# Hippogriff/prifit

Measured on AMD Instinct MI355X. Metric: shapes/sec (fwd+bwd) B=24x2048 pts, PointNet++-MSG+ellipsoid fit, higher is better.
Workload: dtype f32; 1 GPU; configs[2]: PointNet++-MSG + mean-shift(10 it, <=25 clusters) + ellipsoid fit + convex loss, B=24x2048 per GPU, fwd+bwd+Adam; global_batch=24, points=2048, parallelism=dp1, cloud=blobs, embedding=clustered, backbone_grad_param=sa1.conv_blocks.0.0.weight, launch=eager

## Files before the change

### include/prifit_hip.h

```cpp
#ifndef PRIFIT_HIP_H
#define PRIFIT_HIP_H

#include <stdint.h>

#ifdef __cplusplus
extern "C" {
#endif

#define PRIFIT_OK 0
#define PRIFIT_EINVAL (-1)
#define PRIFIT_ELAUNCH (-2)

#define PRIFIT_ABI_VERSION 200
int prifit_version(const char **arch);


int prifit_fps(const float *xyz, int B, int N, int npoint, const int64_t *start_idx,
               int64_t *out_idx, float *new_xyz, void *stream);

int prifit_ball_query(const float *xyz, const float *new_xyz, int B, int N, int S, int R,
                      const float *radius2, const int *nsample, void *const *out, int idx64,
                      void *stream);

int prifit_three_nn(const float *xyz1, const float *xyz2, int B, int N, int S, int32_t *idx,
                    float *dist, float *weight, void *stream);

int prifit_square_distance(const float *src, const float *dst, int B, int S, int N, float *out,
                           void *stream);


int prifit_group_gather(const float *feat, const float *xyz, const float *new_xyz,
                        const int32_t *idx, int B, int N, int S, int K, int C, int order,
                        int ld_out, float *out, void *stream);

int prifit_group_scatter_add(const float *gout, int ld_gout, int col0, const int32_t *idx, int B,
                             int N, int S, int K, int C, float *dfeat, void *stream);

int prifit_pack_cols(const float *w, int rows, int src_cols, const int32_t *map, int dst_cols, float *out, void *stream);
int prifit_unpack_cols(const float *g, int rows, int dst_cols, const int32_t *inv_off, const int32_t *inv_idx, int src_cols,
                       float *gw, void *stream);
int prifit_pack_cols_max_jobs(void);
int prifit_pack_cols_multi(int njobs, const float *const *w, const int32_t *rows, const int32_t *src_cols, const int32_t *const *map,
                           const int32_t *dst_cols, float *const *out, void *stream);
int prifit_unpack_cols_multi(int njobs, const float *const *g, const int32_t *rows, const int32_t *dst_cols, const int32_t *const *inv_off,
                             const int32_t *const *inv_idx, const int32_t *src_cols, float *const *gw, void *stream);

int prifit_three_interpolate(const float *points2, const int32_t *idx, const float *weight, int B,
                             int N, int S, int C, int ld_out, int col0, float *out, void *stream);

int prifit_three_interpolate_bwd(const float *gout, int ld_gout, int col0, const int32_t *idx,
                                 const float *weight, int B, int N, int S, int C, float *dpoints2,
                                 void *stream);
int prifit_fp_rows(const float *points2, const int32_t *idx, const float *weight, const float *points1, int B, int N, int S, int D2,
                   int D1, int kp, float *out, void *stream);


#define PRIFIT_GEMM_NT 0
#define PRIFIT_GEMM_NN 1
#define PRIFIT_GEMM_TN 2
#define PRIFIT_EPI_NONE 0
#define PRIFIT_EPI_CHORD 1
#define PRIFIT_EPI_MSKERNEL 2
#define PRIFIT_EPI_MSBWD 3

int prifit_gemm_f32(int layout, int M, int N, int K, const float *A, long long lda, long long strideA,
                    const float *B, long long ldb, long long strideB, float *C, long long ldc,
                    long long strideC, int batch, int splitk, const float *a_scale,
                    const float *a_shift, const float *b_scale, const float *b_shift,
                    const float *bias, long long bias_batch_stride, float *col_stats, int epilogue,
                    const float *epi_batch_scalar, const float *epi_aux, long long ld_aux,
                    long long stride_aux, const float *epi_row_add, float *a_rowsum, int accumulate, void *stream);

int prifit_chord_sym_f32(const float *A, long long lda, long long strideA, float *C, long long ldc, long long strideC,
                         int n, int K, int batch, unsigned long long *owner_key, void *stream);
int prifit_chord_sym_mask(const float *A, long long lda, long long strideA, const float *thr, uint32_t *mask, int n, int K, int batch,
                          unsigned long long *owner_key, void *stream);
int prifit_gram_sym_f32(const float *A, long long lda, long long strideA, float *C, long long ldc, long long strideC, int n, int K,
                        int batch, void *stream);

int prifit_gemm_pool_f32(int M, int N, int K, const float *A, long long lda, const float *W, long long ldb, float *Y,
                         long long ldc, const float *a_scale, const float *a_shift, const float *bias, float *col_stats,
                         float *cand, void *stream);
int prifit_gemm_pool_supported(int M, int N, int K);

int prifit_gemm_stream_f32(int layout, int M, int N, int K, const float *A, long long lda, const float *B,
                           long long ldb, float *C, long long ldc, const float *a_scale, const float *a_shift,
                           const float *bias, float *col_stats, void *stream);
int prifit_gemm_stream_supported(int layout, int M, int N, int K);
int prifit_gemm_stream_slabs(int M, int K);

int prifit_gemm_dual_nn_f32(int M, int N, int K1, int K2, const float *A1, const float *A2, long long lda,
                            long long strideA, const float *B1, const float *B2, long long ldb, long long strideB,
                            float *C, long long ldc, long long strideC, int batch, int splitk, int accumulate,
                            void *stream);

int prifit_gemm_dgrad_bnred_f32(int M, int N, int K, const float *dY, long long lda, const float *W, long long ldb,
                                float *G, long long ldc, const float *Yprev, long long ldy, const float *scale,
                                const float *shift, const float *mean, const float *invstd, float *red_slab, void *stream);
int prifit_slab_sum(const float *part, int nslab, long long n, float *out, void *stream);
int prifit_global_pool_winners_supported(int Cout, int Cin);
int prifit_global_pool_winners_f32(int Bs, int K, int Cout, int Cin, const int32_t *arg, const float *T, const float *W,
                                   long long ldw, const float *X, long long ldx, float *dX, long long lddx, float *dW,
                                   long long lddw, void *stream);

int prifit_gemm_stream_gather_f32(int M, int N, const int32_t *idx, const float *U, const float *Vc, int n_points, int n_centres,
                                  int rows_per_centre, const float *B, long long ldb, float *C, long long ldc,
                                  const float *a_scale, const float *a_shift, const float *bias, float *col_stats, void *stream);
int prifit_gemm_stream_bwd_gather_f32(long long P, int Cout, const float *G, const float *Y, const float *scale,
                                      const float *shift, const float *coef_a, const float *coef_b, const float *coef_d,
                                      const float *W, long long ldw, const int32_t *idx, const float *U, const float *Vc,
                                      int n_points, int n_centres, int rows_per_centre, const float *p_scale,
                                      const float *p_shift, const float *p_mean, const float *p_invstd, float *Gp, long long ldgp,
                                      float *red_slab, float *dW, long long lddw, float *workspace, void *stream);
int prifit_gemm_stream_pool_f32(int M, int N, int K, const float *A, long long lda, const float *B, long long ldb,
                                float *C, long long ldc, const float *a_scale, const float *a_shift, const float *bias,
                                float *col_stats, float *cand, void *stream);
int prifit_pool_from_candidates(const float *cand, const float *scale, const float *shift, int G, int K, int C,
                                int rows_per_sample, float slope, float *out, long long ldo, int32_t *arg, float *ystar,
                                void *stream);

int prifit_gemm_stream_dgrad_f32(int M, int N, int K, const float *dY, long long lda, const float *W, long long ldb,
                                 float *G, long long ldc, const float *Yprev, long long ldy, const float *scale,
                                 const float *shift, const float *mean, const float *invstd, float *red_slab, void *stream);

int prifit_pool_bwd_table(const float *gp, long long ldgp, const float *Y, long long ldy, const int32_t *arg,
                          const float *scale, const float *shift, const float *coef_a, int G, int K, int C, float slope,
                          float *T, void *stream);
int prifit_gemm_stream_dgrad_pool_f32(int M, int N, int K, const float *Y, long long lda, const float *W, long long ldb,
                                      float *G, long long ldc, const float *bias_dW, const int32_t *pool_arg,
                                      const float *pool_T, const float *coef_b, int pool_K, const float *Yprev,
                                      long long ldy, const float *scale, const float *shift, const float *mean,
                                      const float *invstd, float *red_slab, void *stream);
int prifit_gemm_stream_tn_pool_f32(int Mo, int No, long long P, const float *Y, long long ldy, const float *A,
                                   long long lda, float *out, long long ldo, const float *b_scale,
                                   const float *b_shift, const int32_t *pool_arg, const float *pool_T,
                                   const float *coef_b, const float *coef_d, int pool_K, float *workspace,
                                   void *stream);

int prifit_gemm_stream_tn_bn_f32(int Mo, int No, long long P, const float *G, const float *Y, long long ldy, const float *A,
                                 long long lda, float *out, long long ldo, const float *b_scale, const float *b_shift,
                                 const float *scale, const float *shift, const float *coef_a, const float *coef_b,
                                 const float *coef_d, float *workspace, void *stream);
int prifit_gemm_stream_dgrad_bn_f32(int M, int N, int K, const float *Gin, const float *Y, long long lda, const float *W,
                                    long long ldb, float *G, long long ldc, const float *scale_l, const float *shift_l,
                                    const float *coef_a, const float *coef_b, const float *coef_d, const float *Yprev,
                                    long long ldy, const float *scale, const float *shift, const float *mean,
                                    const float *invstd, float *red_slab, void *stream);
int prifit_gemm_stream_tn_f32(int Mo, int No, long long P, const float *G, long long ldg, const float *A,
                              long long lda, float *out, long long ldo, const float *b_scale,
                              const float *b_shift, float *workspace, void *stream);
long long prifit_gemm_stream_tn_workspace(int Mo, int No, long long P);
int prifit_gemm_stream_tn_supported(int Mo, int No, long long P);

int prifit_gemm_tile_m(int N);
int prifit_gemm_stats_tile_m(int M, int N);


int prifit_reduce_rows_per_slab(void);
int prifit_pool_reduce_groups_per_slab(void);

int prifit_col_stats(const float *Y, long long ld, int P, int C, float *slab, void *stream);
long long prifit_col_sum_workspace(int P, int C);
int prifit_col_sum(const float *Y, long long ld, int P, int C, float *out, float *workspace, void *stream);
int prifit_col_sum_samples(const float *Y, long long ld, int P, int C, int rows_per_sample, float *out, float *workspace,
                           void *stream);

// ... 291 lines not shown
```

### prifit_amd/csrc/gemm.hip

```cpp
#include <stdlib.h>

#include <type_traits>

#include "common.h"

typedef float f32x16 __attribute__((ext_vector_type(16)));

enum { LAY_NT = 0, LAY_NN = 1, LAY_TN = 2 };
enum { EPI_NONE = 0, EPI_CHORD = 1, EPI_MSKERNEL = 2, EPI_MSBWD = 3, EPI_BNRED = 4 };

struct GemmArgs {
    const float *A, *B;
    float *C;
    int M, N, K;
    long long lda, ldb, ldc;
    long long sA, sB, sC;
    int batch, splitk;
    const float *a_scale, *a_shift;
    const float *b_scale, *b_shift;
    const float *bias;
    long long bias_stride;
    float *stats;
    int epi;
    const float *epi_batch_scalar;
    const float *aux;
    const float *row_add;
    float *a_rowsum;
    long long ldaux, sAux;
    const float *red_scale, *red_shift, *red_mean, *red_invstd;
    long long dA2, dB2;
    int kswitch;
    int accumulate;
    int vecA, vecB;
    int ntiles;
    float *cand;
};

#ifndef GEMM_W8
#define GEMM_W8 6
#endif
constexpr int BK = 32;
constexpr int PAD = 4;

__device__ __forceinline__ float4 ld4(const float *p) { return *reinterpret_cast<const float4 *>(p); }

template <int ROWS, bool KC, bool VEC, bool AFF, int NTH>
struct TileLoader {
    static constexpr int NV = ROWS * BK / 4 / NTH;
    static_assert(NV * NTH * 4 == ROWS * BK, "tile must divide evenly over the threads");
    float4 v[NV];
    const float *ptr[NV];
    int klo[NV];
    int c0[NV];
    unsigned okmask[NV];
    long long step;
    int K, R, cclamp;

    __device__ __forceinline__ void init(const float *__restrict__ base, long long ld, int r0, int R_, int K_)
    {
        K = K_; R = R_;
        step = KC ? (long long)BK : (long long)BK * ld;
#pragma unroll
        for (int p = 0; p < NV; ++p) {
            const int id = threadIdx.x + NTH * p;
            if (KC) {
                const int gr = r0 + id / (BK / 4);
                klo[p] = (id % (BK / 4)) * 4;
                okmask[p] = gr < R ? 0xFu : 0u;
                ptr[p] = base + (long long)(gr < R ? gr : 0) * ld + (klo[p] < K ? klo[p] : 0);
                c0[p] = 0;
            } else {
                klo[p] = id / (ROWS / 4);
                const int gr = r0 + (id % (ROWS / 4)) * 4;
                unsigned m = 0;
#pragma unroll
                for (int j = 0; j < 4; ++j) m |= (gr + j < R) ? (1u << j) : 0u;
                okmask[p] = m;
                c0[p] = m ? gr : 0;
                ptr[p] = base + (long long)klo[p] * ld + c0[p];
            }
        }
    }

    int kload;
    __device__ __forceinline__ void load(int k0, const float *__restrict__, const float *__restrict__)
    {
        kload = k0;
        const int kt = k0 / BK;
#pragma unroll
        for (int p = 0; p < NV; ++p) {
            const int gk = k0 + klo[p];
            const bool kin = gk < K;
            const float *src = ptr[p] + (kin ? (long long)kt * step : 0);
            if (!KC && !kin && klo[p] >= K) src = ptr[p] - (long long)klo[p] * (step / BK);
            if (VEC) {
                v[p] = ld4(src);
            } else {
                float e[4];
#pragma unroll
                for (int j = 0; j < 4; ++j) {
                    const bool ok = KC ? (okmask[p] && (gk + j) < K) : (kin && ((okmask[p] >> j) & 1u));
                    e[j] = src[ok ? j : 0];
                }
                v[p] = make_float4(e[0], e[1], e[2], e[3]);
            }
        }
    }

    __device__ __forceinline__ void finish(const float *__restrict__ scale, const float *__restrict__ shift)
    {
#pragma unroll
        for (int p = 0; p < NV; ++p) {
            const int gk = kload + klo[p];
            const bool kin = gk < K;
            float4 x = v[p];
            if (VEC) {
                if (AFF) {
                    const int cc = KC ? (kin ? gk : 0) : c0[p];
                    const float4 s = ld4(scale + cc), t = ld4(shift + cc);
                    x.x = fmaxf(fmaf(x.x, s.x, t.x), 0.f); x.y = fmaxf(fmaf(x.y, s.y, t.y), 0.f);
                    x.z = fmaxf(fmaf(x.z, s.z, t.z), 0.f); x.w = fmaxf(fmaf(x.w, s.w, t.w), 0.f);
                }
                if (!(kin && okmask[p])) x = make_float4(0.f, 0.f, 0.f, 0.f);
            } else {
// ... 607 lines not shown
            const int y_voff = (RED && cok) ? (int)(((long long)rbase * g.ldaux + col) * 4) : 0x7fffffff;
            float kf[16];
            if (RED) {
#pragma unroll
                for (int r = 0; r < 16; ++r) {
                    const int ro = ((r & 3) + 8 * (r >> 2)) * ldy4;
                    kf[r] = __builtin_bit_cast(float, full_rows ? __builtin_amdgcn_raw_buffer_load_b32(yrs, y_voff, ro, 0)
                                                                 : __builtin_amdgcn_raw_buffer_load_b32(yrs, cok ? y_voff + ro : y_voff, 0, 0));
                }
            }
            float vmax = -INFINITY, vmin = INFINITY, v0 = 0.f;
            int imax = 0, imin = 0;
#pragma unroll
            for (int r = 0; r < 16; ++r) {
                const int row = rbase + (r & 3) + 8 * (r >> 2);
                const float v = acc[b][r] + bias;
                const float vs = (cok && (full_rows || row < g.M)) ? v : 0.f;
                if (PMAX) {
                    const int ri = (r & 3) + 8 * (r >> 2) + 4 * lh;
                    const bool rok = full_rows || row < g.M;
                    if (rok && v > vmax) { vmax = v; imax = ri; }
                    if (rok && v < vmin) { vmin = v; imin = ri; }
                }
                if (RED) {
                    const float gm = fmaf(kf[r], rs, rt) > 0.f ? vs : 0.f;
                    csum[b] += gm;
                    csq[b] += gm * ((kf[r] - rmu) * ris);
                } else {
                    csum[b] += vs;
                    if (r == 0) v0 = vs;
                    else if (r == 1) csq[b] = fmaf(v0, v0, vs * vs);
                    else csq[b] = fmaf(vs, vs, csq[b]);
                }
                {
                    const int ro = ((r & 3) + 8 * (r >> 2)) * ldc4;
                    if (full_rows) __builtin_amdgcn_raw_buffer_store_b32(__builtin_bit_cast(unsigned, v), crs, c_voff, ro, 0);
                    else __builtin_amdgcn_raw_buffer_store_b32(__builtin_bit_cast(unsigned, v), crs, cok ? c_voff + ro : c_voff, 0, 0);
                }
            }
            if (PMAX) {
                const float ov = __shfl_xor(vmax, 32, 64), on = __shfl_xor(vmin, 32, 64);
                const int oi = __shfl_xor(imax, 32, 64), oj = __shfl_xor(imin, 32, 64);
                if (ov > vmax || (ov == vmax && oi < imax)) { vmax = ov; imax = oi; }
                if (on < vmin || (on == vmin && oj < imin)) { vmin = on; imin = oj; }
                const int blk_row = m0 + wm0;
                if (lh == 0 && cok && blk_row < g.M) {
                    float *cd = g.cand + (long long)(blk_row >> 5) * 4 * g.N + col;
                    cd[0] = vmax; cd[g.N] = __int_as_float(imax); cd[2 * g.N] = vmin; cd[3 * g.N] = __int_as_float(imin);
                }
            }
        }
        PERS_STAMP(3);
        if (g.stats) {
            float *red = lds;
#pragma unroll
            for (int b = 0; b < TN; ++b) {
                const float s = csum[b] + __shfl_xor(csum[b], 32, 64);
                const float q = csq[b] + __shfl_xor(csq[b], 32, 64);
                if (lh == 0) {
                    red[(wmi * 2 + 0) * BN + wn0 + 32 * b + li] = s;
                    red[(wmi * 2 + 1) * BN + wn0 + 32 * b + li] = q;
                }
            }
            __syncthreads();
            for (int t = threadIdx.x; t < 2 * BN; t += NTH) {
                const int which = t / BN, c = t - which * BN;
                float s = 0.f;
#pragma unroll
                for (int w = 0; w < BM / WM; ++w) s += red[(w * 2 + which) * BN + c];
                if (n0 + c < g.N) g.stats[((long long)tile_m * 2 + which) * g.N + n0 + c] = s;
            }
            if (has_next) __syncthreads();
        }
        PERS_STAMP(4);
        if (!has_next) break;
        tix = ntix; tile_m = ntile_m; tile_n = ntile_n;
        la.finish(g.a_scale, g.a_shift);
        la.store(lds); lb.store(lds + SZA);
        __syncthreads();
        PERS_STAMP(5);
#ifdef PERS_STAMPS
        ++st_tile;
#endif
    }
}

#ifndef CHORD_XCD
#define CHORD_XCD 1
#endif
template <int MODE>
__global__ __launch_bounds__(512) __attribute__((amdgpu_waves_per_eu(4, 4))) void chord_sym_kernel(
    const float *__restrict__ A, long long lda, long long sA, float *__restrict__ C, long long ldc, long long sC, int n, int K,
    int batch, unsigned long long *__restrict__ okey, const float *__restrict__ thr, unsigned *__restrict__ mask)
{
    constexpr bool GRAM = MODE == 1, MASK = MODE == 2;
    constexpr int BM = 128, BN = 128, WM = 32, WN = 64, NTH = 512, TN = WN / 32, WAVES_N = BN / WN;
    constexpr int SZ = BM * (BK + PAD);
    constexpr int TLD = BM + 4;
    __shared__ __attribute__((aligned(16))) float lds[4 * SZ];
    static_assert(4 * SZ >= BN * TLD, "the transposed tile fits the staging buffers");
    const int T = n / BM;
    int t, zb;
#if CHORD_XCD
    xcd_shape_block((int)blockIdx.x, T * (T + 1) / 2, batch, zb, t);
#else
    t = (int)blockIdx.x % (T * (T + 1) / 2); zb = (int)blockIdx.x / (T * (T + 1) / 2);
#endif
    int tile_m = 0;
    while (t >= T - tile_m) { t -= T - tile_m; ++tile_m; }
    const int tile_n = tile_m + t;
    const int m0 = tile_m * BM, n0 = tile_n * BN;
    const float *Az = A + (long long)zb * sA;
    float *Cz = MASK ? nullptr : C + (long long)zb * sC;
    const int MW = n / 32;
    unsigned *Mz = MASK ? mask + (long long)zb * n * MW : nullptr;
    const float th = MASK ? thr[zb] : 0.f;
    const int wave = __builtin_amdgcn_readfirstlane(threadIdx.x >> 6), lane = threadIdx.x & 63;
    const int li = lane & 31, lh = lane >> 5;
    const int wm0 = (wave / WAVES_N) * WM, wn0 = (wave % WAVES_N) * WN;

    BufLoader<BM, true, false, NTH> la, lb;
    la.init(Az, lda, m0, n, K);
    lb.init(Az, lda, n0, n, K);
    const int ktiles = K / BK;
    la.load(0); lb.load(0);
    la.store(lds); lb.store(lds + SZ);
    __syncthreads();
    f32x16 acc[TN];
#pragma unroll
    for (int b = 0; b < TN; ++b)
#pragma unroll
        for (int r = 0; r < 16; ++r) acc[b][r] = 0.f;
    for (int kt = 0; kt < ktiles; ++kt) {
        const int stage = kt & 1;
        const float *As = lds + stage * 2 * SZ, *Bs = As + SZ;
        const bool more = kt + 1 < ktiles;
        if (more) { la.load((kt + 1) * BK); lb.load((kt + 1) * BK); }
#pragma unroll
        for (int gk = 0; gk < BK / 8; ++gk) {
            const float4 fa = read_frag<BM, true>(As, wm0 + li, gk, lh);
            float4 fb[TN];
#pragma unroll
            for (int b = 0; b < TN; ++b) fb[b] = read_frag<BN, true>(Bs, wn0 + 32 * b + li, gk, lh);
#pragma unroll
            for (int b = 0; b < TN; ++b) {
                acc[b] = __builtin_amdgcn_mfma_f32_32x32x2f32(fa.x, fb[b].x, acc[b], 0, 0, 0);
                acc[b] = __builtin_amdgcn_mfma_f32_32x32x2f32(fa.y, fb[b].y, acc[b], 0, 0, 0);
                acc[b] = __builtin_amdgcn_mfma_f32_32x32x2f32(fa.z, fb[b].z, acc[b], 0, 0, 0);
                acc[b] = __builtin_amdgcn_mfma_f32_32x32x2f32(fa.w, fb[b].w, acc[b], 0, 0, 0);
            }
        }
        if (more) {
            float *An = lds + (stage ^ 1) * 2 * SZ;
            la.store(An); lb.store(An + SZ);
        }
        __syncthreads();
    }
    const bool mirror = tile_m != tile_n;
    unsigned long long *okz = okey ? okey + (long long)zb * n : nullptr;
    auto fkey = [](float f) { const unsigned u = __float_as_uint(f); return (u & 0x80000000u) ? ~u : (u | 0x80000000u); };
#pragma unroll
    for (int b = 0; b < TN; ++b) {
        const int col = wn0 + 32 * b + li;
        float cmin = INFINITY;
        int cidx = 0;
#pragma unroll
// ... 82 lines not shown
#pragma unroll
        for (int r = 0; r < 16; ++r) acc[b][r] = 0.f;
    auto step = [&](int kt, auto par) {
        constexpr int S = decltype(par)::value;
        const float *As = lds + S * (SZA + SZB), *Bs = As + SZA;
        if (kt + 2 < kt1) { la[S].load((kt + 2) * BK); lb[S].load((kt + 2) * BK); }
        __builtin_amdgcn_sched_barrier(0);
        mma_ktile<BM, false, BN, false, TN>(As, Bs, wm0 + li, wn0 + li, lh, acc, BK / 8, nbv);
        if (kt + 1 < kt1) {
            float *An = lds + (S ^ 1) * (SZA + SZB);
            lb[S ^ 1].finish(g.b_scale, g.b_shift);
            la[S ^ 1].store(An); lb[S ^ 1].store(An + SZA);
        }
        __syncthreads();
    };
    int kt = kt0;
    for (; kt + 1 < kt1; kt += 2) {
        step(kt, std::integral_constant<int, 0>());
        step(kt + 1, std::integral_constant<int, 1>());
    }
    if (kt < kt1) step(kt, std::integral_constant<int, 0>());
    const int rbase = m0 + wm0 + 4 * lh;
#pragma unroll
    for (int b = 0; b < TN; ++b) {
        const int col = n0 + wn0 + 32 * b + li;
        if (col >= g.N) continue;
#pragma unroll
        for (int r = 0; r < 16; ++r) {
            const int row = rbase + (r & 3) + 8 * (r >> 2);
            if (row >= g.M) continue;
            float *dst = g.C + (long long)row * g.ldc + col;
            if (g.splitk > 1) unsafeAtomicAdd(dst, acc[b][r]);
            else if (g.accumulate) *dst += acc[b][r];
            else *dst = acc[b][r];
        }
    }
}

static bool launch_tnsk(const GemmArgs &g, hipStream_t st)
{
    if (g.batch != 1 || g.a_scale || g.bias || g.stats || g.epi != EPI_NONE || g.a_rowsum || g.kswitch ||
        !(g.vecA && g.vecB) || (g.M & 3) || (g.N & 3) || (g.splitk > 1 && !g.accumulate) || g.splitk > 65535)
        return false;
    const long long lim = 0x7ff00000LL;
    if ((long long)g.K * g.lda * 4 >= lim || (long long)g.K * g.ldb * 4 >= lim) return false;
    const dim3 grid(((g.M + 127) / 128) * ((g.N + 127) / 128), 1, g.splitk), block(512);
    if (g.b_scale) hipLaunchKernelGGL((gemm_tnsk_kernel<true>), grid, block, 0, st, g);
    else hipLaunchKernelGGL((gemm_tnsk_kernel<false>), grid, block, 0, st, g);
    return true;
}

static bool launch_persistent(const GemmArgs &g_, int lay, hipStream_t st, float *want_cand = nullptr, bool dry = false)
{
    GemmArgs g = g_;
    if (lay == LAY_TN || g.batch != 1 || g.splitk != 1 || g.accumulate || g.a_rowsum || g.kswitch ||
        g.b_scale || !(g.epi == EPI_NONE || g.epi == EPI_BNRED) || !(g.vecA && g.vecB) || (g.K & 3) || (lay == LAY_NN && (g.N & 3)))
        return false;
    const long long lim = 0x7ff00000LL;
    if ((long long)g.M * g.lda * 4 >= lim || (long long)(lay == LAY_NT ? g.N : g.K) * g.ldb * 4 >= lim ||
        (long long)g.M * g.ldc * 4 >= lim || (g.epi == EPI_BNRED && (long long)g.M * g.ldaux * 4 >= lim))
        return false;
    g.ntiles = ((g.M + 127) / 128) * ((g.N + 127) / 128);
    const int slots = 512;
    if (g.ntiles <= slots) return false;
    if (dry) return lay == LAY_NT && g.epi == EPI_NONE && g.a_scale;
    const dim3 grid(slots), block(512);
    if (lay == LAY_NT) {
        if (g.epi != EPI_NONE) return false;
        if (want_cand) {
            g.cand = want_cand;
            if (g.a_scale) hipLaunchKernelGGL((gemm_pers_kernel<LAY_NT, true, false, true>), grid, block, 0, st, g);
            else hipLaunchKernelGGL((gemm_pers_kernel<LAY_NT, false, false, true>), grid, block, 0, st, g);
        } else if (g.a_scale) hipLaunchKernelGGL((gemm_pers_kernel<LAY_NT, true, false>), grid, block, 0, st, g);
        else hipLaunchKernelGGL((gemm_pers_kernel<LAY_NT, false, false>), grid, block, 0, st, g);
    } else {
        if (want_cand) return false;
        if (g.a_scale) return false;
        if (g.epi == EPI_BNRED) hipLaunchKernelGGL((gemm_pers_kernel<LAY_NN, false, true>), grid, block, 0, st, g);
        else hipLaunchKernelGGL((gemm_pers_kernel<LAY_NN, false, false>), grid, block, 0, st, g);
    }
    return true;
}

__global__ __launch_bounds__(512, 4) void gemm_dual_sk_kernel(const GemmArgs g)
{
    constexpr int BM = 128, BN = 128, WN = 64, NTH = 512, TN = 2, WAVES_N = 2;
    constexpr int SZA = BM * (BK + PAD), SZB = BK * (BN + PAD);
    __shared__ __attribute__((aligned(16))) float lds[2 * (SZA + SZB)];
    const int tilesM = g.M / BM;
    const int ktiles = g.K / BK;
    const long long total = (long long)g.batch * tilesM * ktiles;
    int u = (int)(total * blockIdx.x / gridDim.x);
    const int uend = (int)(total * (blockIdx.x + 1) / gridDim.x);
    const int wave = threadIdx.x >> 6, lane = threadIdx.x & 63;
    const int li = lane & 31, lh = lane >> 5;
    const int wm0 = (wave / WAVES_N) * 32, wn0 = (wave % WAVES_N) * WN;
    const int kswitch = g.kswitch ? g.kswitch : 0x7fffffff;

    while (u < uend) {
        const int t = u / ktiles;
        const int kt0 = u - t * ktiles, kt1 = min(ktiles, kt0 + (uend - u));
        const int z = t / tilesM, tile_m = t - z * tilesM;
        const int m0 = tile_m * BM;
        const float *A = g.A + (long long)z * g.sA;
        const float *B = g.B + (long long)z * g.sB;
        float *C = g.C + (long long)z * g.sC;

        f32x16 acc[TN];
#pragma unroll
        for (int b = 0; b < TN; ++b)
#pragma unroll
            for (int r = 0; r < 16; ++r) acc[b][r] = 0.f;
        ExactLoader<BM, true, false, NTH> la;
        ExactLoader<BN, false, false, NTH> lb;
        la.init(A, g.lda, m0, g.M, g.K);
        lb.init(B, g.ldb, 0, g.N, g.K);
        if (kt0 >= kswitch) { la.shift(g.dA2); lb.shift(g.dB2); }
        la.load(kt0 * BK, nullptr, nullptr);
        lb.load(kt0 * BK, nullptr, nullptr);
        la.store(lds);
        lb.store(lds + SZA);
        __syncthreads();
        for (int kt = kt0; kt < kt1; ++kt) {
            const int stage = (kt - kt0) & 1;
            const float *As = lds + stage * (SZA + SZB), *Bs = As + SZA;
            const bool more = kt + 1 < kt1;
            if (more) {
                if (kt + 1 == kswitch) { la.shift(g.dA2); lb.shift(g.dB2); }
                la.load((kt + 1) * BK, nullptr, nullptr);
                lb.load((kt + 1) * BK, nullptr, nullptr);
            }
            mma_ktile<BM, true, BN, false, TN>(As, Bs, wm0 + li, wn0 + li, lh, acc);
            if (more) {
                float *An = lds + (stage ^ 1) * (SZA + SZB);
                la.store(An);
                lb.store(An + SZA);
            }
            __syncthreads();
        }
        const int rbase = m0 + wm0 + 4 * lh;
#pragma unroll
        for (int b = 0; b < TN; ++b) {
            const int col = wn0 + 32 * b + li;
#pragma unroll
            for (int r = 0; r < 16; ++r)
                unsafeAtomicAdd(C + (long long)(rbase + (r & 3) + 8 * (r >> 2)) * g.ldc + col, acc[b][r]);
        }
        u += kt1 - kt0;
    }
}

template <int BM, int BN, int WM, int WN, int LAY, bool VEC>
static void launch_aff(const GemmArgs &g, dim3 grid, hipStream_t st)
{
    const dim3 block((BM / WM) * (BN / WN) * 64);
    const long long spanA = (LAY == LAY_TN ? (long long)g.K * g.lda : (long long)g.M * g.lda) * 4;
    const long long spanB = (LAY == LAY_NT ? (long long)g.N * g.ldb : (long long)g.K * g.ldb) * 4;
    const bool exact = VEC && !g.a_rowsum && spanA < 0x7ff00000LL && spanB < 0x7ff00000LL;
    if (exact) {
        if (g.a_scale) hipLaunchKernelGGL((gemm_kernel<BM, BN, WM, WN, LAY, true, true, true, false, true>), grid, block, 0, st, g);
        else if (g.b_scale) hipLaunchKernelGGL((gemm_kernel<BM, BN, WM, WN, LAY, true, true, false, true, true>), grid, block, 0, st, g);
        else hipLaunchKernelGGL((gemm_kernel<BM, BN, WM, WN, LAY, true, true, false, false, true>), grid, block, 0, st, g);
        return;
    }
    if (g.a_scale) hipLaunchKernelGGL((gemm_kernel<BM, BN, WM, WN, LAY, VEC, VEC, true, false>), grid, block, 0, st, g);
    else if (g.b_scale) hipLaunchKernelGGL((gemm_kernel<BM, BN, WM, WN, LAY, VEC, VEC, false, true>), grid, block, 0, st, g);
    else hipLaunchKernelGGL((gemm_kernel<BM, BN, WM, WN, LAY, VEC, VEC, false, false>), grid, block, 0, st, g);
}

template <int BM, int BN, int WM, int WN>
static int launch_cfg(const GemmArgs &g, int lay, hipStream_t st)
{
    const int tilesM = (g.M + BM - 1) / BM, tilesN = (g.N + BN - 1) / BN;
    dim3 grid(tilesM * tilesN, 1, g.batch * g.splitk);
    const bool vec = g.vecA && g.vecB;
    if (g.a_scale && g.b_scale) return PRIFIT_EINVAL;
    switch (lay) {
        case LAY_NT:
            if (vec) launch_aff<BM, BN, WM, WN, LAY_NT, true>(g, grid, st);
            else launch_aff<BM, BN, WM, WN, LAY_NT, false>(g, grid, st);
            break;
        case LAY_NN:
            if (vec) launch_aff<BM, BN, WM, WN, LAY_NN, true>(g, grid, st);
            else launch_aff<BM, BN, WM, WN, LAY_NN, false>(g, grid, st);
            break;
        default:
            if (vec) launch_aff<BM, BN, WM, WN, LAY_TN, true>(g, grid, st);
            else launch_aff<BM, BN, WM, WN, LAY_TN, false>(g, grid, st);
            break;
    }
    return prifit_check_launch();
}

static inline bool aligned16(const void *p) { return ((uintptr_t)p & 15) == 0; }

static inline bool small_tiles(int M, int N, int batch, int splitk)
{
    const long long wgs = (long long)((M + 127) / 128) * ((N + 127) / 128) * batch * splitk;
    return wgs < (splitk > 1 ? 160 : 520) && M > 64 && N > 32;
}

static int dispatch(GemmArgs &g, int layout, void *stream)
{
    const int M = g.M, N = g.N, K = g.K;
    const int extA = layout == LAY_TN ? M : K, extB = layout == LAY_NT ? K : N;
    g.vecA = aligned16(g.A) && (g.lda % 4 == 0) && (g.sA % 4 == 0) && (extA % 4 == 0);
    g.vecB = aligned16(g.B) && (g.ldb % 4 == 0) && (g.sB % 4 == 0) && (extB % 4 == 0);
    hipStream_t st = as_stream(stream);
    if (small_tiles(M, N, g.batch, g.splitk)) return launch_cfg<64, 64, 32, 32>(g, layout, st);
    if (N <= 32) return launch_cfg<128, 32, 32, 32>(g, layout, st);
    if (N <= 64) return launch_cfg<128, 64, 32, 64>(g, layout, st);
    if (N <= 96) return launch_cfg<128, 96, 32, 96>(g, layout, st);
    if (launch_persistent(g, layout, st)) return prifit_check_launch();
    if (layout == LAY_TN && launch_tnsk(g, st)) return prifit_check_launch();
    return launch_cfg<128, 128, 32, 64>(g, layout, st);
}

extern "C" {

#ifdef PERS_STAMPS
int prifit_debug_pers_ktail(int on)
{
    return hipMemcpyToSymbol(HIP_SYMBOL(g_pers_ktail), &on, sizeof(int)) == hipSuccess ? 0 : -1;
}
int prifit_debug_pers_stamps(unsigned long long *host, int n)
{
    return hipMemcpyFromSymbol(host, HIP_SYMBOL(g_pers_stamps), sizeof(unsigned long long) * (size_t)n) == hipSuccess ? 0 : -1;
}
#endif

int prifit_gemm_tile_m(int N)
{
    (void)N;
    return 128;
}

int prifit_gemm_stats_tile_m(int M, int N)
{
    return small_tiles(M, N, 1, 1) ? 64 : 128;
}

int prifit_gemm_f32(int layout, int M, int N, int K, const float *A, long long lda, long long strideA,
                    const float *B, long long ldb, long long strideB, float *C, long long ldc,
                    long long strideC, int batch, int splitk, const float *a_scale, const float *a_shift,
                    const float *b_scale, const float *b_shift, const float *bias, long long bias_batch_stride,
                    float *col_stats, int epilogue, const float *epi_batch_scalar, const float *epi_aux, long long ld_aux,
                    long long stride_aux, const float *epi_row_add, float *a_rowsum, int accumulate, void *stream)
{
    if (!A || !B || !C || M <= 0 || N <= 0 || K <= 0 || batch <= 0 || splitk <= 0 || layout < 0 || layout > 2 ||
        (epilogue != 100 && (epilogue < 0 || epilogue > 3)) || (epilogue >= EPI_MSKERNEL && !epi_batch_scalar) ||
        (epilogue == EPI_MSBWD && !epi_aux) || (splitk > 1 && !accumulate) ||
        ((a_scale == nullptr) != (a_shift == nullptr)) || ((b_scale == nullptr) != (b_shift == nullptr)) ||
        (col_stats && (batch != 1 || splitk != 1)) || (epilogue != EPI_NONE && epilogue != 100 && splitk != 1) || (long long)batch * splitk > 65535)
        return PRIFIT_EINVAL;
    GemmArgs g;
    g.A = A; g.B = B; g.C = C; g.M = M; g.N = N; g.K = K;
    g.lda = lda; g.ldb = ldb; g.ldc = ldc; g.sA = strideA; g.sB = strideB; g.sC = strideC;
    g.batch = batch; g.splitk = splitk;
    g.a_scale = a_scale; g.a_shift = a_shift; g.b_scale = b_scale; g.b_shift = b_shift;
    g.bias = bias; g.bias_stride = bias_batch_stride; g.stats = col_stats; g.epi = epilogue; g.epi_batch_scalar = epi_batch_scalar;
    g.accumulate = accumulate; g.aux = epi_aux; g.ldaux = ld_aux; g.sAux = stride_aux;
    g.row_add = epi_row_add; g.a_rowsum = a_rowsum;
    g.red_scale = g.red_shift = g.red_mean = g.red_invstd = nullptr;
    g.dA2 = g.dB2 = 0; g.kswitch = 0;
    if (a_rowsum && (layout == LAY_TN || splitk != 1)) return PRIFIT_EINVAL;
    return dispatch(g, layout, stream);
}

int prifit_gemm_dual_nn_f32(int M, int N, int K1, int K2, const float *A1, const float *A2, long long lda,
                            long long strideA, const float *B1, const float *B2, long long ldb, long long strideB,
                            float *C, long long ldc, long long strideC, int batch, int splitk, int accumulate,
                            void *stream)
{
    if (!A1 || !A2 || !B1 || !B2 || !C || M <= 0 || N <= 0 || K1 <= 0 || K2 <= 0 || (K1 % BK) || batch <= 0 ||
        splitk <= 0 || (splitk > 1 && !accumulate) || (long long)batch * splitk > 65535 || lda < K1 || lda < K2 ||
        ldb < N || ldc < N)
        return PRIFIT_EINVAL;
    if ((((uintptr_t)A1 ^ (uintptr_t)A2) | ((uintptr_t)B1 ^ (uintptr_t)B2)) & 15) return PRIFIT_EINVAL;
    GemmArgs g;
    g.A = A1; g.B = B1; g.C = C; g.M = M; g.N = N; g.K = K1 + K2;
    g.lda = lda; g.ldb = ldb; g.ldc = ldc; g.sA = strideA; g.sB = strideB; g.sC = strideC;
    g.batch = batch; g.splitk = splitk;
    g.a_scale = g.a_shift = g.b_scale = g.b_shift = nullptr;
    g.bias = nullptr; g.bias_stride = 0; g.stats = nullptr; g.epi = EPI_NONE; g.epi_batch_scalar = nullptr;
    g.accumulate = accumulate; g.aux = nullptr; g.ldaux = 0; g.sAux = 0; g.row_add = nullptr; g.a_rowsum = nullptr;
    g.red_scale = g.red_shift = g.red_mean = g.red_invstd = nullptr;
    g.dA2 = (A2 - A1) - (long long)K1;
    g.dB2 = (B2 - B1) - (long long)K1 * ldb;
    g.kswitch = K1 / BK;
    if (accumulate && N == 128 && M % 128 == 0 && K1 == K2 && aligned16(A1) && aligned16(B1) && (lda % 4 == 0) &&
        (ldb % 4 == 0) && (strideA % 4 == 0) && (strideB % 4 == 0) && (long long)M * lda * 4 < 0x7ff00000LL &&
        (long long)(K1 + K2) * ldb * 4 < 0x7ff00000LL) {
        static const int slots = [] {
            int dev = 0;
            hipDeviceProp_t p;
            if (hipGetDevice(&dev) != hipSuccess || hipGetDeviceProperties(&p, dev) != hipSuccess) return 512;
            return 2 * p.multiProcessorCount;
        }();
        const long long total = (long long)batch * (M / 128) * ((K1 + K2) / BK);
        const int grid = (int)(total < slots ? total : slots);
        hipLaunchKernelGGL(gemm_dual_sk_kernel, dim3(grid), dim3(512), 0, as_stream(stream), g);
        return prifit_check_launch();
    }
    return dispatch(g, LAY_NN, stream);
}

int prifit_gemm_dgrad_bnred_f32(int M, int N, int K, const float *dY, long long lda, const float *W, long long ldb,
                                float *G, long long ldc, const float *Yprev, long long ldy, const float *scale,
                                const float *shift, const float *mean, const float *invstd, float *red_slab, void *stream)
{
    if (!dY || !W || !G || !Yprev || !scale || !shift || !mean || !invstd || !red_slab || M <= 0 || N <= 0 || K <= 0 ||
        lda < K || ldb < N || ldc < N || ldy < N)
        return PRIFIT_EINVAL;
    GemmArgs g;
    g.A = dY; g.B = W; g.C = G; g.M = M; g.N = N; g.K = K;
    g.lda = lda; g.ldb = ldb; g.ldc = ldc; g.sA = g.sB = g.sC = 0;
    g.batch = 1; g.splitk = 1;
    g.a_scale = g.a_shift = g.b_scale = g.b_shift = nullptr;
    g.bias = nullptr; g.bias_stride = 0; g.stats = red_slab; g.epi = EPI_BNRED; g.epi_batch_scalar = nullptr;
    g.accumulate = 0; g.aux = Yprev; g.ldaux = ldy; g.sAux = 0; g.row_add = nullptr; g.a_rowsum = nullptr;
    g.red_scale = scale; g.red_shift = shift; g.red_mean = mean; g.red_invstd = invstd;
    g.dA2 = g.dB2 = 0; g.kswitch = 0;
    return dispatch(g, LAY_NN, stream);
}

int prifit_chord_sym_f32(const float *A, long long lda, long long strideA, float *C, long long ldc, long long strideC,
                         int n, int K, int batch, unsigned long long *owner_key, void *stream)
{
    if (!A || !C || n <= 0 || (n % 128) || K <= 0 || (K % BK) || batch <= 0 || batch > 65535 || lda < K || ldc < n || (lda & 3) ||
        (ldc & 3) || (strideA & 3) || (strideC & 3) || ((uintptr_t)A & 15) || ((uintptr_t)C & 15) ||
        (long long)n * lda * 4 >= 0x7ff00000LL)
        return PRIFIT_EINVAL;
    const int T = n / 128;
    hipLaunchKernelGGL(chord_sym_kernel<0>, dim3((unsigned)(T * (T + 1) / 2 * batch)), dim3(512), 0, as_stream(stream), A, lda,
                       strideA, C, ldc, strideC, n, K, batch, owner_key, (const float *)nullptr, (unsigned *)nullptr);
    return prifit_check_launch();
}

int prifit_chord_sym_mask(const float *A, long long lda, long long strideA, const float *thr, uint32_t *mask, int n, int K, int batch,
                          unsigned long long *owner_key, void *stream)
{
    if (!A || !thr || !mask || n <= 0 || (n % 128) || K <= 0 || (K % BK) || batch <= 0 || batch > 65535 || lda < K || (lda & 3) ||
        (strideA & 3) || ((uintptr_t)A & 15) || (long long)n * lda * 4 >= 0x7ff00000LL)
        return PRIFIT_EINVAL;
    const int T = n / 128;
    hipLaunchKernelGGL(chord_sym_kernel<2>, dim3((unsigned)(T * (T + 1) / 2 * batch)), dim3(512), 0, as_stream(stream), A, lda,
                       strideA, (float *)nullptr, 0LL, 0LL, n, K, batch, owner_key, thr, mask);
    return prifit_check_launch();
}

int prifit_gram_sym_f32(const float *A, long long lda, long long strideA, float *C, long long ldc, long long strideC, int n, int K,
                        int batch, void *stream)
{
    if (!A || !C || n <= 0 || (n % 128) || K <= 0 || (K % BK) || batch <= 0 || batch > 65535 || lda < K || ldc < n || (lda & 3) ||
        (ldc & 3) || (strideA & 3) || (strideC & 3) || ((uintptr_t)A & 15) || ((uintptr_t)C & 15) ||
        (long long)n * lda * 4 >= 0x7ff00000LL)
        return PRIFIT_EINVAL;
    const int T = n / 128;
    hipLaunchKernelGGL(chord_sym_kernel<1>, dim3((unsigned)(T * (T + 1) / 2 * batch)), dim3(512), 0, as_stream(stream), A, lda,
                       strideA, C, ldc, strideC, n, K, batch, (unsigned long long *)nullptr, (const float *)nullptr, (unsigned *)nullptr);
    return prifit_check_launch();
}

static void pool_gemm_args(GemmArgs &g, int M, int N, int K, const float *A, long long lda, const float *W, long long ldb,
                           float *Y, long long ldc, const float *a_scale, const float *a_shift, const float *bias, float *stats)
{
    g.A = A; g.B = W; g.C = Y; g.M = M; g.N = N; g.K = K; g.lda = lda; g.ldb = ldb; g.ldc = ldc;
    g.sA = g.sB = g.sC = 0; g.batch = 1; g.splitk = 1;
    g.a_scale = a_scale; g.a_shift = a_shift; g.b_scale = g.b_shift = nullptr;
    g.bias = bias; g.bias_stride = 0; g.stats = stats; g.epi = EPI_NONE; g.epi_batch_scalar = nullptr;
    g.aux = nullptr; g.row_add = nullptr; g.a_rowsum = nullptr; g.ldaux = 0; g.sAux = 0;
    g.red_scale = g.red_shift = g.red_mean = g.red_invstd = nullptr;
    g.dA2 = g.dB2 = 0; g.kswitch = 0; g.accumulate = 0;
    g.vecA = aligned16(A) && (lda % 4 == 0) && (K % 4 == 0);
    g.vecB = aligned16(W) && (ldb % 4 == 0) && (K % 4 == 0);
}

int prifit_gemm_pool_supported(int M, int N, int K)
{
    if (M <= 0 || N <= 96 || K <= 0 || (M & 31)) return 0;
    GemmArgs g;
    static float dummy[4] __attribute__((aligned(16)));
    pool_gemm_args(g, M, N, K, dummy, K, dummy, K, dummy, N, dummy, dummy, nullptr, nullptr);
    return launch_persistent(g, LAY_NT, nullptr, nullptr, true) ? 1 : 0;
}

int prifit_gemm_pool_f32(int M, int N, int K, const float *A, long long lda, const float *W, long long ldb, float *Y,
                         long long ldc, const float *a_scale, const float *a_shift, const float *bias, float *col_stats,
                         float *cand, void *stream)
{
    if (!A || !W || ((a_scale == nullptr) != (a_shift == nullptr)) || !cand || !prifit_gemm_pool_supported(M, N, K) ||
        lda < K || ldb < K || ldc < N)
        return PRIFIT_EINVAL;
    GemmArgs g;
    pool_gemm_args(g, M, N, K, A, lda, W, ldb, Y, ldc, a_scale, a_shift, bias, col_stats);
    if (!launch_persistent(g, LAY_NT, as_stream(stream), cand)) return PRIFIT_EINVAL;
    return prifit_check_launch();
}

}
```

Baseline: 1640 shapes/s.

## Add weight-resident persistent GEMM kernel for tall skinny MLP layers

Adds a persistent GEMM kernel that keeps the whole weight matrix (N up to 256, K up to 256) resident in LDS and streams 128-row slabs of A straight from global memory into MFMA registers. Columns are partitioned into classes spread across CUs per XCD, so each CU reloads only its own weight slice once. It handles the NT and NN layouts, fused BN-affine+ReLU on inputs, column stats, BN-reduce backward, and pool candidate epilogues. It is dispatched for very tall GEMMs (M >= 131072) before the existing paths. The trade-off is heavy LDS use limiting occupancy to 2 waves per EU, and the first-load pass per CU is serialized.

New measurement: 1633 shapes/s. No clear change (-0.4%).

```diff
diff --git a/include/prifit_hip.h b/include/prifit_hip.h
--- a/include/prifit_hip.h
+++ b/include/prifit_hip.h
@@ -11,7 +11,7 @@
 #define PRIFIT_EINVAL (-1)
 #define PRIFIT_ELAUNCH (-2)
 
-#define PRIFIT_ABI_VERSION 200
+#define PRIFIT_ABI_VERSION 201
 int prifit_version(const char **arch);
 
 
@@ -82,6 +82,8 @@
                          long long ldc, const float *a_scale, const float *a_shift, const float *bias, float *col_stats,
                          float *cand, void *stream);
 int prifit_gemm_pool_supported(int M, int N, int K);
+
+int prifit_gemm_resident_supported(int layout, int M, int N, int K);
 
 int prifit_gemm_stream_f32(int layout, int M, int N, int K, const float *A, long long lda, const float *B,
                            long long ldb, float *C, long long ldc, const float *a_scale, const float *a_shift,
diff --git a/prifit_amd/csrc/gemm.hip b/prifit_amd/csrc/gemm.hip
--- a/prifit_amd/csrc/gemm.hip
+++ b/prifit_amd/csrc/gemm.hip
@@ -40,6 +40,9 @@
 #define GEMM_W8 6
 #endif
 constexpr int BK = 32;
+#ifndef RES_MIN_ROWS
+#define RES_MIN_ROWS 131072
+#endif
 constexpr int PAD = 4;
 
 __device__ __forceinline__ float4 ld4(const float *p) { return *reinterpret_cast<const float4 *>(p); }
@@ -813,6 +816,261 @@
 #ifdef PERS_STAMPS
         ++st_tile;
 #endif
+    }
+}
+
+struct ResPlan {
+    int ncls, ld, slabs;
+    int col0[8], nb[8], pos0[9];
+};
+
+#ifdef PERS_STAMPS
+#define RES_STAMP(i)                                                                                        \
+    do {                                                                                                     \
+        if (st_slot >= 0 && st_tile < 8) {                                                                   \
+            const unsigned long long t_ = __builtin_amdgcn_s_memtime();                                      \
+            if (threadIdx.x == 0) g_pers_stamps[(st_slot * 8 + st_tile) * 8 + (i)] = t_;                    \
+        }                                                                                                    \
+    } while (0)
+#else
+#define RES_STAMP(i) do { } while (0)
+#endif
+
+template <int LAY, bool FA, bool RED, bool PMAX = false>
+__global__ __launch_bounds__(512) __attribute__((amdgpu_waves_per_eu(2, 2))) void gemm_res_kernel(const GemmArgs g, const ResPlan p)
+{
+#ifdef PERS_STAMPS
+    const int st_slot = (blockIdx.x % 31 == 0 && blockIdx.x / 31 < 8) ? (int)blockIdx.x / 31 : -1;
+    int st_tile = 0;
+    RES_STAMP(6);
+#endif
+    constexpr int TN = 4, NTH = 512, OOBV = 0x7fffffff;
+    extern __shared__ __attribute__((aligned(16))) float rlds[];
+    const int xcd = blockIdx.x & 7, pos = blockIdx.x >> 3;
+    int col0 = p.col0[0], nb = p.nb[0], p0 = p.pos0[0], p1 = p.pos0[1];
+#pragma unroll
+    for (int c = 1; c < 8; ++c)
+        if (c < p.ncls && pos >= p.pos0[c]) { col0 = p.col0[c]; nb = p.nb[c]; p0 = p.pos0[c]; p1 = p.pos0[c + 1]; }
+    const int ld = p.ld;
+
+    float *Bs = rlds, *sc = rlds + nb * 32 * ld, *sh = sc + ld;
+    if (LAY == LAY_NT) {
+        const int ldq = ld >> 2;
+        for (int i = threadIdx.x; i < nb * 32 * ldq; i += NTH) {
+            const int c = i / ldq, k = 4 * (i - c * ldq);
+            float4 v = make_float4(0.f, 0.f, 0.f, 0.f);
+            if (col0 + c < g.N && k < g.K) v = ld4(g.B + (long long)(col0 + c) * g.ldb + k);
+            *reinterpret_cast<float4 *>(Bs + c * ld + k) = v;
+        }
+    } else {
+        const int nq = nb * 8;
+        for (int i = threadIdx.x; i < ld * nq; i += NTH) {
+            const int k = i / nq, c = 4 * (i - k * nq);
+            float4 v = make_float4(0.f, 0.f, 0.f, 0.f);
+            if (k < g.K && col0 + c < g.N) v = ld4(g.B + (long long)k * g.ldb + col0 + c);
+            Bs[c * ld + k] = v.x; Bs[(c + 1) * ld + k] = v.y; Bs[(c + 2) * ld + k] = v.z; Bs[(c + 3) * ld + k] = v.w;
+        }
+    }
+    if (FA)
+        for (int i = threadIdx.x; i < ld; i += NTH) { sc[i] = i < g.K ? g.a_scale[i] : 0.f; sh[i] = i < g.K ? g.a_shift[i] : 0.f; }
+    __syncthreads();
+    RES_STAMP(7);
+
+    const int wave = __builtin_amdgcn_readfirstlane(threadIdx.x >> 6), lane = threadIdx.x & 63;
+    const int li = lane & 31, lh = lane >> 5;
+    if (wave < 4) __builtin_amdgcn_s_setprio(1);
+    const int Wc = (p1 - p0) * 8;
+    int t = (pos - p0) * 8 + wave;
+    if (xcd + 8 * t >= p.slabs) return;
+    const int nch = (g.K + 31) >> 5;
+    const int ngk_last = (g.K - (nch - 1) * 32 + 7) >> 3;
+
+    const __amdgpu_buffer_rsrc_t ars = __builtin_amdgcn_make_buffer_rsrc(const_cast<float *>(g.A), 0, 0x7ffffffc, 0x00020000);
+    const __amdgpu_buffer_rsrc_t crs = __builtin_amdgcn_make_buffer_rsrc(g.C, 0, g.C ? (int)((long long)g.M * g.ldc * 4) : 0, 0x00020000);
+    const __amdgpu_buffer_rsrc_t yrs = __builtin_amdgcn_make_buffer_rsrc(
+        const_cast<float *>(RED ? g.aux : nullptr), 0, RED ? (int)((long long)g.M * g.ldaux * 4) : 0, 0x00020000);
+    const int ldc4 = (int)g.ldc * 4, ldy4 = RED ? (int)g.ldaux * 4 : 0;
+
+    const float *Bl = Bs + li * ld + 4 * lh;
+    auto rdB = [&](float4 (&f)[TN], int k0) {
+#pragma unroll
+        for (int b = 0; b < TN; ++b)
+            if (b < nb) f[b] = *reinterpret_cast<const float4 *>(Bl + 32 * b * ld + k0);
+    };
+    auto rowoff = [&](int row0) { return row0 + li < g.M ? (int)(((long long)(row0 + li) * g.lda + 4 * lh) * 4) : OOBV; };
+    auto ldA = [&](float4 (&f)[4], int voff, int c) {
+        const int k0 = 32 * c;
+        if (k0 + 32 <= g.K) {
+#pragma unroll
+            for (int q = 0; q < 4; ++q) {
+                const f32x4v v = __builtin_bit_cast(f32x4v, __builtin_amdgcn_raw_buffer_load_b128(ars, voff + 32 * q, k0 * 4, 0));
+                f[q] = make_float4(v.x, v.y, v.z, v.w);
+            }
+        } else {
+#pragma unroll
+            for (int q = 0; q < 4; ++q) {
+                const int vo = (voff != OOBV && k0 + 8 * q + 4 * lh < g.K) ? voff + 32 * q : OOBV;
+                const f32x4v v = __builtin_bit_cast(f32x4v, __builtin_amdgcn_raw_buffer_load_b128(ars, vo, k0 * 4, 0));
+                f[q] = make_float4(v.x, v.y, v.z, v.w);
+            }
+        }
+    };
+
+    auto ldY = [&](float (&y)[16], int b, int rb, bool full, int pitch4) {
+        const int col = col0 + 32 * b + li;
+        const bool cok = col < g.N;
+        const int y_voff = cok ? (int)(((long long)rb * g.ldaux + col) * 4) : OOBV;
+#pragma unroll
+        for (int r = 0; r < 16; ++r) {
+            const int ro = ((r & 3) + 8 * (r >> 2)) * pitch4;
+            y[r] = __builtin_bit_cast(float, full ? __builtin_amdgcn_raw_buffer_load_b32(yrs, y_voff, ro, 0)
+                                                  : __builtin_amdgcn_raw_buffer_load_b32(yrs, cok ? y_voff + ro : y_voff, 0, 0));
+        }
+    };
+    int row0 = (xcd + 8 * t) * 128, blk = 0;
+    int voff = rowoff(row0);
+    float4 fa[4], fan[4], fb[2][TN];
+    ldA(fan, voff, 0);
+    rdB(fb[0], 0);
+    float ssum[TN], ssq[TN];
+#pragma unroll
+    for (int b = 0; b < TN; ++b) { ssum[b] = 0.f; ssq[b] = 0.f; }
+
+    for (;;) {
+        RES_STAMP(0);
+        int nblk = blk + 1, nt = t, nrow0 = row0 + 32;
+        if (nblk == 4 || nrow0 >= g.M) { nblk = 0; nt = t + Wc; nrow0 = (xcd + 8 * nt) * 128; }
+        const bool has_next = xcd + 8 * nt < p.slabs;
+        const int nvoff = has_next ? rowoff(nrow0) : OOBV;
+        const bool full_rows = row0 + 32 <= g.M;
+        const int rbase = row0 + 4 * lh;
+        int ldc4b = ldc4, ldy4b = ldy4;
+        asm volatile("" : "+s"(ldc4b), "+s"(ldy4b));
+        f32x16 acc[TN];
+#pragma unroll
+        for (int b = 0; b < TN; ++b)
+#pragma unroll
+            for (int r = 0; r < 16; ++r) acc[b][r] = 0.f;
+        float kf[2][16];
+
+        for (int c = 0; c < nch; ++c) {
+            const bool last = c + 1 == nch;
+#pragma unroll
+            for (int q = 0; q < 4; ++q) fa[q] = fan[q];
+            ldA(fan, last ? nvoff : voff, last ? 0 : c + 1);
+            if (RED && last) ldY(kf[0], 0, rbase, full_rows, ldy4b);
+            if (FA) {
+#pragma unroll
+                for (int q = 0; q < 4; ++q) {
+                    const int k = 32 * c + 8 * q + 4 * lh;
+                    const int kc = k < g.K ? k : 0;
+                    const float4 s = *reinterpret_cast<const float4 *>(sc + kc), h = *reinterpret_cast<const float4 *>(sh + kc);
+                    float4 x = fa[q];
+                    x.x = fmaxf(fmaf(x.x, s.x, h.x), 0.f); x.y = fmaxf(fmaf(x.y, s.y, h.y), 0.f);
+                    x.z = fmaxf(fmaf(x.z, s.z, h.z), 0.f); x.w = fmaxf(fmaf(x.w, s.w, h.w), 0.f);
+                    fa[q] = (voff != OOBV && k < g.K) ? x : make_float4(0.f, 0.f, 0.f, 0.f);
+                }
+            }
+            const int ngk = last ? ngk_last : 4;
+            const int kn = last ? 0 : 32 * (c + 1);
+#pragma unroll
+            for (int gk = 0; gk < 4; ++gk) {
+                if (gk > 0 && gk >= ngk) break;
+                if (gk + 1 < 4) { if (gk + 1 < ngk) rdB(fb[(gk + 1) & 1], 32 * c + 8 * (gk + 1)); }
+                else rdB(fb[0], kn);
+                __builtin_amdgcn_sched_barrier(0);
+                const float4 a = fa[gk];
+#pragma unroll
+                for (int b = 0; b < TN; ++b) {
+                    if (b >= nb) continue;
+                    const float4 w = fb[gk & 1][b];
+                    acc[b] = __builtin_amdgcn_mfma_f32_32x32x2f32(a.x, w.x, acc[b], 0, 0, 0);
+                    acc[b] = __builtin_amdgcn_mfma_f32_32x32x2f32(a.y, w.y, acc[b], 0, 0, 0);
+                    acc[b] = __builtin_amdgcn_mfma_f32_32x32x2f32(a.z, w.z, acc[b], 0, 0, 0);
+                    acc[b] = __builtin_amdgcn_mfma_f32_32x32x2f32(a.w, w.w, acc[b], 0, 0, 0);
+                }
+                __builtin_amdgcn_sched_barrier(0);
+            }
+            if (ngk < 4) rdB(fb[0], kn);
+        }
+        RES_STAMP(1);
+
+#pragma unroll
+        for (int b = 0; b < TN; ++b) {
+            if (b >= nb) continue;
+            if (RED && b + 1 < nb) ldY(kf[(b + 1) & 1], b + 1, rbase, full_rows, ldy4b);
+            float csum = 0.f, csq = 0.f;
+            const int col = col0 + 32 * b + li;
+            const bool cok = col < g.N;
+            const float bias = (g.bias && cok) ? g.bias[col] : 0.f;
+            float rs = 0.f, rt = 0.f, rmu = 0.f, ris = 0.f;
+            if (RED && cok) { rs = g.red_scale[col]; rt = g.red_shift[col]; rmu = g.red_mean[col]; ris = g.red_invstd[col]; }
+            const int c_voff = cok ? (int)(((long long)rbase * g.ldc + col) * 4) : OOBV;
+            float vmax = -INFINITY, vmin = INFINITY, v0 = 0.f;
+            int imax = 0, imin = 0;
+#pragma unroll
+            for (int r = 0; r < 16; ++r) {
+                const int row = rbase + (r & 3) + 8 * (r >> 2);
+                const float v = acc[b][r] + bias;
+                const float vs = (cok && (full_rows || row < g.M)) ? v : 0.f;
+                if (PMAX) {
+                    const int ri = (r & 3) + 8 * (r >> 2) + 4 * lh;
+                    const bool rok = full_rows || row < g.M;
+                    if (rok && v > vmax) { vmax = v; imax = ri; }
+                    if (rok && v < vmin) { vmin = v; imin = ri; }
+                }
+                if (RED) {
+                    const float y = kf[b & 1][r];
+                    const float gm = fmaf(y, rs, rt) > 0.f ? vs : 0.f;
+                    csum += gm;
+                    csq += gm * ((y - rmu) * ris);
+                } else {
+                    csum += vs;
+                    if (r == 0) v0 = vs;
+                    else if (r == 1) csq = fmaf(v0, v0, vs * vs);
+                    else csq = fmaf(vs, vs, csq);
+                }
+                {
+                    const int ro = ((r & 3) + 8 * (r >> 2)) * ldc4b;
+                    if (full_rows) __builtin_amdgcn_raw_buffer_store_b32(__builtin_bit_cast(unsigned, v), crs, c_voff, ro, 0);
+                    else __builtin_amdgcn_raw_buffer_store_b32(__builtin_bit_cast(unsigned, v), crs, cok ? c_voff + ro : c_voff, 0, 0);
+                }
+            }
+            if (PMAX) {
+                const float ov = __shfl_xor(vmax, 32, 64), on = __shfl_xor(vmin, 32, 64);
+                const int oi = __shfl_xor(imax, 32, 64), oj = __shfl_xor(imin, 32, 64);
+                if (ov > vmax || (ov == vmax && oi < imax)) { vmax = ov; imax = oi; }
+                if (on < vmin || (on == vmin && oj < imin)) { vmin = on; imin = oj; }
+                if (lh == 0 && cok) {
+                    float *cd = g.cand + (long long)(row0 >> 5) * 4 * g.N + col;
+                    cd[0] = vmax; cd[g.N] = __int_as_float(imax); cd[2 * g.N] = vmin; cd[3 * g.N] = __int_as_float(imin);
+                }
+            }
+            ssum[b] += csum + __shfl_xor(csum, 32, 64);
+            ssq[b] += csq + __shfl_xor(csq, 32, 64);
+            if (RED) __builtin_amdgcn_sched_barrier(0);
+        }
+        if (nblk == 0 && g.stats) {
+#pragma unroll
+            for (int b = 0; b < TN; ++b) {
+                if (b >= nb) continue;
+                const int col = col0 + 32 * b + li;
+                if (lh == 0 && col < g.N) {
+                    float *sd = g.stats + (long long)(row0 >> 7) * 2 * g.N + col;
+                    sd[0] = ssum[b]; sd[g.N] = ssq[b];
+                }
+            }
+        }
+        if (nblk == 0) {
+#pragma unroll
+            for (int b = 0; b < TN; ++b) { ssum[b] = 0.f; ssq[b] = 0.f; }
+        }
+        RES_STAMP(2);
+#ifdef PERS_STAMPS
+        ++st_tile;
+#endif
+        if (!has_next) break;
+        blk = nblk; t = nt; row0 = nrow0; voff = nvoff;
     }
 }
 
@@ -1061,6 +1319,83 @@
     return true;
 }
 
+static bool res_plan(const GemmArgs &g, int cus, ResPlan &best, size_t &lds)
+{
+    const int per_xcd = cus / 8, nblocks = (g.N + 31) / 32, slabs = (g.M + 127) / 128, T = (slabs + 7) / 8;
+    int ld = (g.K + 7) & ~7;
+    while (((ld >> 2) & 1) == 0) ld += 4;
+    long long best_time = -1;
+    for (int w = 4; w >= 2; w -= 2) {
+        ResPlan p;
+        p.ncls = (nblocks + w - 1) / w; p.ld = ld; p.slabs = slabs;
+        if (p.ncls > 8 || p.ncls > per_xcd || (size_t)(w * 32 + 2) * ld * 4 > 160 * 1024) continue;
+        int n[8];
+        for (int c = 0; c < p.ncls; ++c) { p.col0[c] = c * w * 32; p.nb[c] = nblocks - c * w < w ? nblocks - c * w : w; n[c] = 1; }
+        for (int left = per_xcd - p.ncls; left > 0; --left) {
+            int m = 0;
+            for (int c = 1; c < p.ncls; ++c) if (p.nb[c] * n[m] > p.nb[m] * n[c]) m = c;
+            ++n[m];
+        }
+        long long time = 0;
+        p.pos0[0] = 0;
+        for (int c = 0; c < p.ncls; ++c) {
+            p.pos0[c + 1] = p.pos0[c] + n[c];
+            const long long tc = (long long)((T + 8 * n[c] - 1) / (8 * n[c])) * p.nb[c];
+            if (tc > time) time = tc;
+        }
+        for (int c = p.ncls; c < 8; ++c) { p.col0[c] = 0; p.nb[c] = 0; p.pos0[c + 1] = p.pos0[p.ncls]; }
+        if (best_time < 0 || time < best_time) { best_time = time; best = p; lds = (size_t)(w * 32 + 2) * ld * 4; }
+    }
+    return best_time >= 0;
+}
+
+static bool launch_resident(const GemmArgs &g, int lay, hipStream_t st, float *want_cand = nullptr, bool dry = false)
+{
+#ifdef PRIFIT_NO_RESIDENT
+    return false;
+#endif
+    if (lay == LAY_TN || g.batch != 1 || g.splitk != 1 || g.accumulate || g.a_rowsum || g.kswitch || g.b_scale ||
+        !(g.epi == EPI_NONE || g.epi == EPI_BNRED) || !(g.vecA && g.vecB) || (g.K & 3) || (lay == LAY_NN && (g.N & 3)))
+        return false;
+    if (lay == LAY_NT ? g.epi != EPI_NONE : (want_cand || g.a_scale)) return false;
+    if (g.N <= 64 || g.N > 256 || g.K < 32 || g.K > 256 || g.M < RES_MIN_ROWS) return false;
+    const long long lim = 0x7ff00000LL;
+    if ((long long)g.M * g.lda * 4 >= lim || (long long)g.M * g.ldc * 4 >= lim || (g.epi == EPI_BNRED && (long long)g.M * g.ldaux * 4 >= lim))
+        return false;
+    static const int cus = [] {
+        int dev = 0;
+        hipDeviceProp_t prop;
+        if (hipGetDevice(&dev) != hipSuccess || hipGetDeviceProperties(&prop, dev) != hipSuccess) return 256;
+        return prop.multiProcessorCount;
+    }();
+    if (cus < 64 || (cus & 7)) return false;
+    ResPlan p;
+    size_t lds = 0;
+    if (!res_plan(g, cus, p, lds)) return false;
+    if (dry) return true;
+    if (lds < 84 * 1024) lds = 84 * 1024;
+    GemmArgs a = g;
+    a.cand = want_cand;
+    const dim3 grid(cus), block(512);
+#define RES_LAUNCH(...)                                                                                              \
+    do {                                                                                                             \
+        static const hipError_t attr = hipFuncSetAttribute(reinterpret_cast<const void *>(&gemm_res_kernel<__VA_ARGS__>), \
+                                                           hipFuncAttributeMaxDynamicSharedMemorySize, 160 * 1024);  \
+        if (attr != hipSuccess) return false;                                                                        \
+        hipLaunchKernelGGL((gemm_res_kernel<__VA_ARGS__>), grid, block, lds, st, a, p);                              \
+    } while (0)
+    if (lay == LAY_NT) {
+        if (want_cand) { if (g.a_scale) RES_LAUNCH(LAY_NT, true, false, true); else RES_LAUNCH(LAY_NT, false, false, true); }
+        else if (g.a_scale) RES_LAUNCH(LAY_NT, true, false);
+        else RES_LAUNCH(LAY_NT, false, false);
+    } else {
+        if (g.epi == EPI_BNRED) RES_LAUNCH(LAY_NN, false, true);
+        else RES_LAUNCH(LAY_NN, false, false);
+    }
+#undef RES_LAUNCH
+    return true;
+}
+
 __global__ __launch_bounds__(512, 4) void gemm_dual_sk_kernel(const GemmArgs g)
 {
     constexpr int BM = 128, BN = 128, WN = 64, NTH = 512, TN = 2, WAVES_N = 2;
@@ -1189,6 +1524,7 @@
     if (small_tiles(M, N, g.batch, g.splitk)) return launch_cfg<64, 64, 32, 32>(g, layout, st);
     if (N <= 32) return launch_cfg<128, 32, 32, 32>(g, layout, st);
     if (N <= 64) return launch_cfg<128, 64, 32, 64>(g, layout, st);
+    if (launch_resident(g, layout, st)) return prifit_check_launch();
     if (N <= 96) return launch_cfg<128, 96, 32, 96>(g, layout, st);
     if (launch_persistent(g, layout, st)) return prifit_check_launch();
     if (layout == LAY_TN && launch_tnsk(g, st)) return prifit_check_launch();
@@ -1355,6 +1691,16 @@
     g.vecB = aligned16(W) && (ldb % 4 == 0) && (K % 4 == 0);
 }
 
+int prifit_gemm_resident_supported(int layout, int M, int N, int K)
+{
+    if ((layout != LAY_NT && layout != LAY_NN) || M <= 0 || N <= 0 || K <= 0) return 0;
+    GemmArgs g;
+    static float dummy[4] __attribute__((aligned(16)));
+    pool_gemm_args(g, M, N, K, dummy, K, dummy, layout == LAY_NT ? K : N, dummy, N, nullptr, nullptr, nullptr, nullptr);
+    g.vecB = (layout == LAY_NT ? K : N) % 4 == 0;
+    return launch_resident(g, layout, nullptr, nullptr, true) ? 1 : 0;
+}
+
 int prifit_gemm_pool_supported(int M, int N, int K)
 {
     if (M <= 0 || N <= 96 || K <= 0 || (M & 31)) return 0;
@@ -1373,7 +1719,7 @@
         return PRIFIT_EINVAL;
     GemmArgs g;
     pool_gemm_args(g, M, N, K, A, lda, W, ldb, Y, ldc, a_scale, a_shift, bias, col_stats);
-    if (!launch_persistent(g, LAY_NT, as_stream(stream), cand)) return PRIFIT_EINVAL;
+    if (!launch_resident(g, LAY_NT, as_stream(stream), cand) && !launch_persistent(g, LAY_NT, as_stream(stream), cand)) return PRIFIT_EINVAL;
     return prifit_check_launch();
 }
 
```
